# TaoMiner/joint-kg-recommender

Hardware: NVIDIA H100
Metric: scored (h,r,t) triples/s, TransE d=100 forward + margin loss + backward (higher is better)
Workload: dtype f32

## Files before the change

### joint-kg-recommender_b200/csrc/common.cuh

```cuda
#pragma once
#include <cuda_runtime.h>
#include <stdint.h>
#include "../../include/kgrec_b200.h"

namespace kgrec {

constexpr unsigned FULL = 0xffffffffu;
constexpr int kWarpsPerCta = 8;
constexpr int kThreads = kWarpsPerCta * 32;
constexpr int kMaxPref = 128;

void set_error(const char* fmt, ...);
#define KGREC_CUDA_OK(expr)                                                        \
  do {                                                                             \
    cudaError_t e__ = (expr);                                                      \
    if (e__ != cudaSuccess) {                                                      \
      kgrec::set_error("%s failed: %s (%s:%d)", #expr, cudaGetErrorString(e__),    \
                       __FILE__, __LINE__);                                        \
      return KGREC_ERR_CUDA;                                                       \
    }                                                                              \
  } while (0)
int sm_count();
float l2_keep_fraction(double table_bytes);

__device__ __forceinline__ float warp_sum(float v) {
#pragma unroll
  for (int o = 16; o > 0; o >>= 1) v += __shfl_xor_sync(FULL, v, o);
  return v;
}
__device__ __forceinline__ void warp_sum2(float& a, float& b) {
#pragma unroll
  for (int o = 16; o > 0; o >>= 1) {
    a += __shfl_xor_sync(FULL, a, o);
    b += __shfl_xor_sync(FULL, b, o);
  }
}
__device__ __forceinline__ float warp_max(float v) {
#pragma unroll
  for (int o = 16; o > 0; o >>= 1) v = fmaxf(v, __shfl_xor_sync(FULL, v, o));
  return v;
}

__device__ __forceinline__ float warp_reduce_scatter8(float (&v)[8], int lane) {
#pragma unroll
  for (int o = 16, n = 4; n > 0; o >>= 1, n >>= 1) {
    const bool up = (lane & o) != 0;
#pragma unroll
    for (int j = 0; j < 4; ++j) {
      if (j < n) {
        const float send = up ? v[j] : v[j + n];
        const float keep = up ? v[j + n] : v[j];
        v[j] = keep + __shfl_xor_sync(FULL, send, o);
      }
    }
  }
  float r = v[0];
  r += __shfl_xor_sync(FULL, r, 2);
  r += __shfl_xor_sync(FULL, r, 1);
  return r;
}

__device__ __forceinline__ int64_t load_idx(const void* p, int64_t i, int is64) {
  return is64 ? __ldg(reinterpret_cast<const long long*>(p) + i)
              : static_cast<int64_t>(__ldg(reinterpret_cast<const int*>(p) + i));
}
__device__ __forceinline__ int64_t checked(int64_t row, int64_t rows, int32_t* status) {
  if (static_cast<uint64_t>(row) >= static_cast<uint64_t>(rows)) {
    if (status) *status = 1;
    return 0;
  }
  return row;
}

__device__ __forceinline__ float4 ldg_f4(const float4* p) {
  float4 r;
  asm volatile("ld.global.nc.L1::no_allocate.v4.f32 {%0,%1,%2,%3}, [%4];"
               : "=f"(r.x), "=f"(r.y), "=f"(r.z), "=f"(r.w) : "l"(p));
  return r;
}
__device__ __forceinline__ void red_add_f4(float* p, float a, float b, float c, float d) {
  asm volatile("red.global.add.v4.f32 [%0], {%1,%2,%3,%4};" ::"l"(p), "f"(a), "f"(b), "f"(c), "f"(d)
               : "memory");
}

__device__ __forceinline__ void prefetch_l1(const void* p) { asm volatile("prefetch.global.L1 [%0];" ::"l"(p)); }

__device__ __forceinline__ uint32_t smem_u32(const void* p) { return static_cast<uint32_t>(__cvta_generic_to_shared(p)); }
__device__ __forceinline__ void mbar_init(uint64_t* bar, uint32_t count) {
  asm volatile("mbarrier.init.shared::cta.b64 [%0], %1;" ::"r"(smem_u32(bar)), "r"(count));
}
__device__ __forceinline__ void mbar_fence_init() { asm volatile("fence.mbarrier_init.release.cluster;" ::: "memory"); }
__device__ __forceinline__ void mbar_arrive(uint64_t* bar) {
  asm volatile("mbarrier.arrive.shared::cta.b64 _, [%0];" ::"r"(smem_u32(bar)) : "memory");
}
__device__ __forceinline__ void mbar_arrive_expect_tx(uint64_t* bar, uint32_t bytes) {
  asm volatile("mbarrier.arrive.expect_tx.shared::cta.b64 _, [%0], %1;" ::"r"(smem_u32(bar)), "r"(bytes) : "memory");
}
__device__ __forceinline__ bool mbar_try_wait(uint64_t* bar, uint32_t parity, uint32_t suspend_ns) {
  uint32_t ok;
  asm volatile(
      "{\n\t.reg .pred p;\n\t"
      "mbarrier.try_wait.parity.shared::cta.b64 p, [%1], %2, %3;\n\t"
      "selp.u32 %0, 1, 0, p;\n\t}"
      : "=r"(ok) : "r"(smem_u32(bar)), "r"(parity), "r"(suspend_ns) : "memory");
  return ok != 0;
}
__device__ __forceinline__ void mbar_wait(uint64_t* bar, uint32_t parity) {
  while (!mbar_try_wait(bar, parity, 20000u)) {}
}
__device__ __forceinline__ void bulk_g2s(void* dst, const void* src, uint32_t bytes, uint64_t* bar) {
  asm volatile("cp.async.bulk.shared::cluster.global.mbarrier::complete_tx::bytes [%0], [%1], %2, [%3];" ::"r"(
                   smem_u32(dst)),
               "l"(src), "r"(bytes), "r"(smem_u32(bar))
               : "memory");
}

__device__ __forceinline__ void fence_proxy_async_smem() { asm volatile("fence.proxy.async.shared::cta;" ::: "memory"); }
__device__ __forceinline__ float4 lds_f4(uint32_t addr) {
  float4 r;
  asm volatile("ld.shared.v4.f32 {%0,%1,%2,%3}, [%4];" : "=f"(r.x), "=f"(r.y), "=f"(r.z), "=f"(r.w) : "r"(addr));
  return r;
}

__device__ __forceinline__ uint64_t policy_evict_last(float fraction) {
  uint64_t p;
  asm volatile("createpolicy.fractional.L2::evict_last.L2::evict_unchanged.b64 %0, %1;" : "=l"(p) : "f"(fraction));
  return p;
}
__device__ __forceinline__ uint64_t policy_evict_first() {
  uint64_t p;
  asm volatile("createpolicy.fractional.L2::evict_first.b64 %0, 1.0;" : "=l"(p));
  return p;
}
__device__ __forceinline__ float4 ldg_f4_hint(const float4* p, uint64_t pol) {
  float4 r;
  asm volatile("ld.global.nc.L1::no_allocate.L2::cache_hint.v4.f32 {%0,%1,%2,%3}, [%4], %5;"
               : "=f"(r.x), "=f"(r.y), "=f"(r.z), "=f"(r.w) : "l"(p), "l"(pol));
  return r;
}
__device__ __forceinline__ void stg_f4_hint(float4* p, float a, float b, float c, float d, uint64_t pol) {
  asm volatile("st.global.L2::cache_hint.v4.f32 [%0], {%1,%2,%3,%4}, %5;" ::"l"(p), "f"(a), "f"(b), "f"(c), "f"(d), "l"(pol)
               : "memory");
}

template <int NCH, bool VEC>
struct Row {
  static constexpr int NE = NCH * 4;
  __device__ __forceinline__ static int elem(int lane, int e) {
    return VEC ? ((lane + 32 * (e >> 2)) * 4 + (e & 3)) : (lane + 32 * e);
  }
  __device__ __forceinline__ static void load(float (&v)[NE], const float* __restrict__ row, int d, int lane) {
    if (VEC) {
#pragma unroll
      for (int i = 0; i < NCH; ++i) {
        const int c = lane + 32 * i;
        float4 t = make_float4(0.f, 0.f, 0.f, 0.f);
        if (c * 4 < d) t = ldg_f4(reinterpret_cast<const float4*>(row) + c);
        v[4 * i] = t.x; v[4 * i + 1] = t.y; v[4 * i + 2] = t.z; v[4 * i + 3] = t.w;
      }
    } else {
#pragma unroll
      for (int e = 0; e < NE; ++e) {
        const int j = lane + 32 * e;
        v[e] = (j < d) ? __ldg(row + j) : 0.f;
      }
    }
  }
  __device__ __forceinline__ static void load_hint(float (&v)[NE], const float* __restrict__ row, int d, int lane, uint64_t pol) {
    static_assert(VEC, "cache-hinted loads are built for the 128-bit path");
#pragma unroll
    for (int i = 0; i < NCH; ++i) {
      const int c = lane + 32 * i;
      float4 t = make_float4(0.f, 0.f, 0.f, 0.f);
      if (c * 4 < d) t = ldg_f4_hint(reinterpret_cast<const float4*>(row) + c, pol);
      v[4 * i] = t.x; v[4 * i + 1] = t.y; v[4 * i + 2] = t.z; v[4 * i + 3] = t.w;
    }
  }
  __device__ __forceinline__ static void store_hint(float* __restrict__ row, const float (&v)[NE], int d, int lane, uint64_t pol) {
    static_assert(VEC, "cache-hinted stores are built for the 128-bit path");
#pragma unroll
    for (int i = 0; i < NCH; ++i) {
      const int c = lane + 32 * i;
      if (c * 4 < d) stg_f4_hint(reinterpret_cast<float4*>(row) + c, v[4 * i], v[4 * i + 1], v[4 * i + 2], v[4 * i + 3], pol);
    }
  }
  __device__ __forceinline__ static void load_s(float (&v)[NE], const float* row, int d, int lane) {
    if (VEC) {
#pragma unroll
      for (int i = 0; i < NCH; ++i) {
        const int c = lane + 32 * i;
        float4 t = make_float4(0.f, 0.f, 0.f, 0.f);
        if (c * 4 < d) t = reinterpret_cast<const float4*>(row)[c];
        v[4 * i] = t.x; v[4 * i + 1] = t.y; v[4 * i + 2] = t.z; v[4 * i + 3] = t.w;
      }
    } else {
#pragma unroll
      for (int e = 0; e < NE; ++e) {
        const int j = lane + 32 * e;
// ... 115 lines not shown
```

### joint-kg-recommender_b200/csrc/train_group.cu

```cuda
#include <cstdlib>
#include "train_dev.cuh"

namespace kgrec {

struct GroupArgs {
  kgrec_tables T;
  const void *ph, *pt, *pr;
  int is64;
  const int32_t* corrupt;
  LossCfg L;
  float keep;
};

__device__ __forceinline__ const float* row_ptr(const float* base, uint32_t row, uint32_t ld) {
  return base + static_cast<uint64_t>(row) * ld;
}

template <int FAM, int NCH>
struct GroupPos {
  using R = Row<NCH, true>;
  static constexpr int NE = R::NE;
  float h[NE], t[NE], w[NE];
  float base_h[NE];
  float base_t[NE];
// ... 466 lines not shown
        cpos += tt > 0.f ? 1.f : 0.f;
      } else {
        const float xx = prm * (sp - sn);
        lsum += fmaxf(-xx, 0.f) + log1pf(expf(-fabsf(xx)));
        const float dp = -prm / (1.f + expf(xx));
        cpos += dp;
        coef = dp * up;
      }
      if (FWD) return;
      const bool regx = REG && nx2 > 1.f;
      if (coef != 0.f || regx) {
        float4 gc = z4;
        if (coef != 0.f) {
          if (L1) {
            gc = make_float4(coef * ddist_term(e.x, 1), coef * ddist_term(e.y, 1), coef * ddist_term(e.z, 1), coef * ddist_term(e.w, 1));
          } else {
            const float c2 = 2.f * coef;
            gc = make_float4(c2 * e.x, c2 * e.y, c2 * e.z, c2 * e.w);
          }
          if (head) { accH.x -= gc.x; accH.y -= gc.y; accH.z -= gc.z; accH.w -= gc.w; }
          else { accT.x -= gc.x; accT.y -= gc.y; accT.z -= gc.z; accT.w -= gc.w; }
        }
        if (regx) { gc.x = fmaf(r2, x.x, gc.x); gc.y = fmaf(r2, x.y, gc.y); gc.z = fmaf(r2, x.z, gc.z); gc.w = fmaf(r2, x.w, gc.w); }
        if (act) {
          if (DENSE) red_add_f4(reinterpret_cast<float*>(gent_b + static_cast<uint64_t>(id) * d4), gc.x, gc.y, gc.z, gc.w);
          else stg_f4_hint(reinterpret_cast<float4*>(gent_b + goff), gc.x, gc.y, gc.z, gc.w, pol_stream);
        }
      } else if (!DENSE) {
        if (act) stg_f4_hint(reinterpret_cast<float4*>(gent_b + goff), 0.f, 0.f, 0.f, 0.f, pol_stream);
      }
      goff += d4;
    };

    for (int k = 0; k < K; k += 2) {
      if (k + 1 < K) {
        idb = ent_id(__shfl_sync(FULL, cv, k + 1), headb);
        if (act) xb = ldg_f4_hint(row(ent_b, idb), pol_keep);
      }
      negative(xa, heada, ida, k);
      if (k + 1 < K) {
        if (k + 2 < K) {
          ida = ent_id(__shfl_sync(FULL, cv, k + 2), heada);
          if (act) xa = ldg_f4_hint(row(ent_b, ida), pol_keep);
        }
        negative(xb, headb, idb, k + 1);
      }
    }
    const float cp = cpos * up;
    const float4 eps = make_float4(cp * ddist_term(ep.x, L1), cp * ddist_term(ep.y, L1), cp * ddist_term(ep.z, L1), cp * ddist_term(ep.w, L1));
    float4 gh = make_float4(accT.x + eps.x, accT.y + eps.y, accT.z + eps.z, accT.w + eps.w);
    float4 gt = make_float4(accH.x - eps.x, accH.y - eps.y, accH.z - eps.z, accH.w - eps.w);
    float4 gr = make_float4(accT.x - accH.x + eps.x, accT.y - accH.y + eps.y, accT.z - accH.z + eps.z, accT.w - accH.w + eps.w);
    if (REG) {
      const float mh = 1.f + n_tail, mt = 1.f + (static_cast<float>(K) - n_tail), mr = 1.f + static_cast<float>(K);
      lreg += mh * fmaxf(nh2 - 1.f, 0.f) + mt * fmaxf(nt2 - 1.f, 0.f) + mr * fmaxf(nr2 - 1.f, 0.f);
      const float ch = nh2 > 1.f ? mh * r2 : 0.f, ct = nt2 > 1.f ? mt * r2 : 0.f, cr = nr2 > 1.f ? mr * r2 : 0.f;
      gh.x = fmaf(ch, h.x, gh.x); gh.y = fmaf(ch, h.y, gh.y); gh.z = fmaf(ch, h.z, gh.z); gh.w = fmaf(ch, h.w, gh.w);
      gt.x = fmaf(ct, t.x, gt.x); gt.y = fmaf(ct, t.y, gt.y); gt.z = fmaf(ct, t.z, gt.z); gt.w = fmaf(ct, t.w, gt.w);
      gr.x = fmaf(cr, r.x, gr.x); gr.y = fmaf(cr, r.y, gr.y); gr.z = fmaf(cr, r.z, gr.z); gr.w = fmaf(cr, r.w, gr.w);
    }
    if (!BWD) {
      if (lane == 0) {
        pos_scores[j] = sp;
        group_loss[j] = lsum + (REG ? lreg : 0.f);
      }
      if (lane < K) neg_scores[static_cast<uint32_t>(j) * K + lane] = mys;
    }
    if (!FWD && act) {
      if (DENSE) {
        red_add_f4(reinterpret_cast<float*>(gent_b + static_cast<uint64_t>(ih0) * d4), gh.x, gh.y, gh.z, gh.w);
        red_add_f4(reinterpret_cast<float*>(gent_b + static_cast<uint64_t>(it0) * d4), gt.x, gt.y, gt.z, gt.w);
        red_add_f4(reinterpret_cast<float*>(grel_b + static_cast<uint64_t>(ir0) * d4), gr.x, gr.y, gr.z, gr.w);
      } else {
        const uint32_t g0 = static_cast<uint32_t>(j) * (2 + K) * d4;
        stg_f4_hint(reinterpret_cast<float4*>(gent_b + g0), gh.x, gh.y, gh.z, gh.w, pol_stream);
        stg_f4_hint(reinterpret_cast<float4*>(gent_b + g0 + d4), gt.x, gt.y, gt.z, gt.w, pol_stream);
        stg_f4_hint(reinterpret_cast<float4*>(grel_b + static_cast<uint32_t>(j) * d4), gr.x, gr.y, gr.z, gr.w, pol_stream);
      }
    }
  }
  if (bad && status) *status = 1;
}

template <bool L1, bool DENSE, bool MARGIN, int W>
__global__ void __launch_bounds__(W * 32, 1)
k_group_step_e_tma(const GroupArgs G, const float up0, float* __restrict__ pos_scores, float* __restrict__ neg_scores,
                   float* __restrict__ group_loss, const kgrec_grads Gr, int64_t* __restrict__ slot_ent,
                   int64_t* __restrict__ slot_rel, int32_t* status, const int S) {
  extern __shared__ __align__(128) unsigned char smem_raw[];
  const kgrec_tables& T = G.T;
  const LossCfg& L = G.L;
  const int lane = threadIdx.x & 31, wid = threadIdx.x >> 5;
  const int K = L.n_neg, n_rows = 3 + K;
  const int n_pos = static_cast<int>(L.n_pos);
  const uint32_t n_ent = static_cast<uint32_t>(T.n_ent);
  const uint32_t ld4 = static_cast<uint32_t>(T.ld) * 4u, d4 = static_cast<uint32_t>(T.dim) * 4u;
  const int bp = static_cast<int>(L.batch_pos < 0x7fffffff ? L.batch_pos : 0x7fffffff);
  const uint64_t pol_stream = policy_evict_first();
  const bool act = lane * 4 < T.dim;
  uint64_t* bars = reinterpret_cast<uint64_t*>(smem_raw) + wid * S;
  int32_t* ids_ring = reinterpret_cast<int32_t*>(smem_raw + static_cast<size_t>(W) * S * 8) + wid * S * 32;
  const uint32_t stage_bytes = static_cast<uint32_t>(n_rows) * d4;
  unsigned char* rows_base = smem_raw + ((static_cast<size_t>(W) * S * (8 + 128) + 127) & ~static_cast<size_t>(127)) +
                             static_cast<size_t>(wid) * S * stage_bytes;
  if (lane == 0)
    for (int s = 0; s < S; ++s) mbar_init(bars + s, 1);
  mbar_fence_init();
  __syncwarp();
  char* gent_b = reinterpret_cast<char*>(Gr.ent) + lane * 16;
  char* grel_b = reinterpret_cast<char*>(Gr.rel) + lane * 16;
  const float prm = L.param;
  const int stride = gridDim.x * W;
  const float4 z4 = make_float4(0.f, 0.f, 0.f, 0.f);
  bool bad = false;
  const void* pcol = lane == 0 ? G.ph : (lane == 1 ? G.pt : G.pr);

  auto issue = [&](int jj, int s) {
    int32_t v = 0;
    if (lane < 3) {
      const int64_t pv = load_idx(pcol, jj, G.is64);
      const int64_t lim = lane == 2 ? T.n_rel : T.n_ent;
      if (static_cast<uint64_t>(pv) >= static_cast<uint64_t>(lim)) bad = true; else v = static_cast<int32_t>(pv);
    } else if (lane < n_rows) {
      v = __ldg(G.corrupt + static_cast<uint32_t>(jj) * K + (lane - 3));
      const uint32_t id = static_cast<uint32_t>(v < 0 ? ~v : v);
      if (id >= n_ent) { bad = true; v = 0; }
    }
    ids_ring[s * 32 + lane] = v;
    if (lane == 0) mbar_arrive_expect_tx(bars + s, stage_bytes);
    __syncwarp();
    if (lane < n_rows) {
      const uint32_t id = lane < 3 ? static_cast<uint32_t>(v) : static_cast<uint32_t>(v < 0 ? ~v : v);
      const char* src = reinterpret_cast<const char*>(lane == 2 ? T.rel : T.ent) + static_cast<uint64_t>(id) * ld4;
      bulk_g2s(rows_base + static_cast<size_t>(s) * stage_bytes + static_cast<size_t>(lane) * d4, src, d4, bars + s);
    }
  };

  int j = blockIdx.x * W + wid;
  for (int s = 0, jj = j; s < S - 1 && jj < n_pos; ++s, jj += stride) issue(jj, s);
  for (int it = 0; j < n_pos; j += stride, ++it) {
    const int s = it % S;
    {
      const int jn = j + (S - 1) * stride;
      if (jn < n_pos) {
        fence_proxy_async_smem();
        __syncwarp();
        issue(jn, (it + S - 1) % S);
      }
    }
    mbar_wait(bars + s, static_cast<uint32_t>(it / S) & 1u);
    const int32_t myid = ids_ring[s * 32 + lane];
    const uint32_t st_addr = smem_u32(rows_base + static_cast<size_t>(s) * stage_bytes) + lane * 16;
    const uint32_t ih0 = static_cast<uint32_t>(__shfl_sync(FULL, myid, 0)), it0 = static_cast<uint32_t>(__shfl_sync(FULL, myid, 1)),
                   ir0 = static_cast<uint32_t>(__shfl_sync(FULL, myid, 2));
    if (slot_ent) {
      const uint32_t s0 = static_cast<uint32_t>(j) * (2 + K);
      if (lane < 2) slot_ent[s0 + lane] = myid;
      if (lane == 2) slot_rel[j] = myid;
      if (lane >= 3 && lane < n_rows) slot_ent[s0 + lane - 1] = myid < 0 ? ~myid : myid;
    }
    float4 h = z4, t = z4, r = z4;
    if (act) { h = lds_f4(st_addr); t = lds_f4(st_addr + d4); r = lds_f4(st_addr + 2 * d4); }
    float up = up0;
    if (!MARGIN) {
      const int b = j / bp;
      up /= static_cast<float>(min(bp, n_pos - b * bp)) * static_cast<float>(K);
    }
    const float4 bh = make_float4(h.x + r.x, h.y + r.y, h.z + r.z, h.w + r.w);
    const float4 bt = make_float4(t.x - r.x, t.y - r.y, t.z - r.z, t.w - r.w);
    const float4 ep = make_float4(bh.x - t.x, bh.y - t.y, bh.z - t.z, bh.w - t.w);
    const float sp = warp_sum(dist_term(ep.x, L1) + dist_term(ep.y, L1) + dist_term(ep.z, L1) + dist_term(ep.w, L1));
    float lsum = 0.f, cpos = 0.f, mys = 0.f;
    float4 accT = z4, accH = z4;
    uint32_t goff = (static_cast<uint32_t>(j) * (2 + K) + 2) * d4;
#pragma unroll 2
    for (int k = 0; k < K; ++k) {
      const int32_t c = __shfl_sync(FULL, myid, 3 + k);
      const bool head = c < 0;
      const uint32_t id = static_cast<uint32_t>(head ? ~c : c);
      float4 x = z4;
      if (act) x = lds_f4(st_addr + (3 + k) * d4);
      const float4 B = head ? bt : bh;
      const float4 e = make_float4(B.x - x.x, B.y - x.y, B.z - x.z, B.w - x.w);
      const float sn = warp_sum(L1 ? fabsf(e.x) + fabsf(e.y) + fabsf(e.z) + fabsf(e.w)
                                   : __fmaf_rn(e.w, e.w, __fmaf_rn(e.z, e.z, __fmaf_rn(e.x, e.x, __fmul_rn(e.y, e.y)))));
      if (lane == k) mys = sn;
      float coef;
      if (MARGIN) {
        const float tt = sp - sn + prm;
        lsum += fmaxf(tt, 0.f);
        coef = tt > 0.f ? up : 0.f;
        cpos += tt > 0.f ? 1.f : 0.f;
      } else {
        const float xx = prm * (sp - sn);
        lsum += fmaxf(-xx, 0.f) + log1pf(expf(-fabsf(xx)));
        const float dp = -prm / (1.f + expf(xx));
        cpos += dp;
        coef = dp * up;
      }
      if (coef != 0.f) {
        float4 gc;
        if (L1) {
          gc = make_float4(coef * ddist_term(e.x, 1), coef * ddist_term(e.y, 1), coef * ddist_term(e.z, 1), coef * ddist_term(e.w, 1));
        } else {
          const float c2 = 2.f * coef;
          gc = make_float4(c2 * e.x, c2 * e.y, c2 * e.z, c2 * e.w);
        }
        if (head) { accH.x -= gc.x; accH.y -= gc.y; accH.z -= gc.z; accH.w -= gc.w; }
        else { accT.x -= gc.x; accT.y -= gc.y; accT.z -= gc.z; accT.w -= gc.w; }
        if (act) {
          if (DENSE) red_add_f4(reinterpret_cast<float*>(gent_b + static_cast<uint64_t>(id) * d4), gc.x, gc.y, gc.z, gc.w);
          else stg_f4_hint(reinterpret_cast<float4*>(gent_b + goff), gc.x, gc.y, gc.z, gc.w, pol_stream);
        }
      } else if (!DENSE) {
        if (act) stg_f4_hint(reinterpret_cast<float4*>(gent_b + goff), 0.f, 0.f, 0.f, 0.f, pol_stream);
      }
      goff += d4;
    }
    const float cp = cpos * up;
    const float4 eps = make_float4(cp * ddist_term(ep.x, L1), cp * ddist_term(ep.y, L1), cp * ddist_term(ep.z, L1), cp * ddist_term(ep.w, L1));
    const float4 gh = make_float4(accT.x + eps.x, accT.y + eps.y, accT.z + eps.z, accT.w + eps.w);
    const float4 gt = make_float4(accH.x - eps.x, accH.y - eps.y, accH.z - eps.z, accH.w - eps.w);
    const float4 gr = make_float4(accT.x - accH.x + eps.x, accT.y - accH.y + eps.y, accT.z - accH.z + eps.z, accT.w - accH.w + eps.w);
    if (lane == 0) {
      pos_scores[j] = sp;
      group_loss[j] = lsum;
    }
    if (lane < K) neg_scores[static_cast<uint32_t>(j) * K + lane] = mys;
    if (act) {
      if (DENSE) {
        red_add_f4(reinterpret_cast<float*>(gent_b + static_cast<uint64_t>(ih0) * d4), gh.x, gh.y, gh.z, gh.w);
        red_add_f4(reinterpret_cast<float*>(gent_b + static_cast<uint64_t>(it0) * d4), gt.x, gt.y, gt.z, gt.w);
        red_add_f4(reinterpret_cast<float*>(grel_b + static_cast<uint64_t>(ir0) * d4), gr.x, gr.y, gr.z, gr.w);
      } else {
        const uint32_t g0 = static_cast<uint32_t>(j) * (2 + K) * d4;
        stg_f4_hint(reinterpret_cast<float4*>(gent_b + g0), gh.x, gh.y, gh.z, gh.w, pol_stream);
        stg_f4_hint(reinterpret_cast<float4*>(gent_b + g0 + d4), gt.x, gt.y, gt.z, gt.w, pol_stream);
        stg_f4_hint(reinterpret_cast<float4*>(grel_b + static_cast<uint32_t>(j) * d4), gr.x, gr.y, gr.z, gr.w, pol_stream);
      }
    }
  }
  if (bad && status) *status = 1;
}

template <bool L1, bool DENSE, bool MARGIN, int MINB, bool PF, bool REG, bool BWD, bool FWD = false>
__global__ void __launch_bounds__(kThreads, MINB)
k_group_step_h(const GroupArgs G, const float up0, const float* __restrict__ up_dev, float* __restrict__ pos_scores,
               float* __restrict__ neg_scores, float* __restrict__ group_loss, const kgrec_grads Gr,
               int64_t* __restrict__ slot_ent, int64_t* __restrict__ slot_rel, int32_t* status) {
  const kgrec_tables& T = G.T;
  const LossCfg& L = G.L;
  const int lane = threadIdx.x & 31, wid = threadIdx.x >> 5;
  const int K = L.n_neg;
  const int n_pos = static_cast<int>(L.n_pos);
  const uint32_t n_ent = static_cast<uint32_t>(T.n_ent);
  const uint32_t ld4 = static_cast<uint32_t>(T.ld) * 4u, d4 = static_cast<uint32_t>(T.dim) * 4u;
  const int bp = static_cast<int>(L.batch_pos < 0x7fffffff ? L.batch_pos : 0x7fffffff);
  const uint64_t pol_keep = policy_evict_last(G.keep), pol_stream = policy_evict_first();
  const bool act = lane * 4 < T.dim;
  const char* ent_b = reinterpret_cast<const char*>(T.ent) + lane * 16;
  const char* rel_b = reinterpret_cast<const char*>(T.rel) + lane * 16;
  const char* nrm_b = reinterpret_cast<const char*>(T.norm) + lane * 16;
  char* gent_b = reinterpret_cast<char*>(Gr.ent) + lane * 16;
  char* grel_b = reinterpret_cast<char*>(Gr.rel) + lane * 16;
  char* gnrm_b = reinterpret_cast<char*>(Gr.norm) + lane * 16;
  const float prm = L.param;
  const int stride = gridDim.x * kWarpsPerCta;
  const float4 z4 = make_float4(0.f, 0.f, 0.f, 0.f);
  auto row = [&](const char* base, uint32_t id) { return reinterpret_cast<const float4*>(base + static_cast<uint64_t>(id) * ld4); };
  auto dot4 = [](const float4& a, const float4& b) { return fmaf(a.x, b.x, fmaf(a.y, b.y, fmaf(a.z, b.z, a.w * b.w))); };
  bool bad = false;
  auto ent_id = [&](int32_t c, bool& head) {
    head = c < 0;
    uint32_t id = static_cast<uint32_t>(head ? ~c : c);
    if (id >= n_ent) { bad = true; id = 0; }
    return id;
  };
  int j = blockIdx.x * kWarpsPerCta + wid;
  const void* pcol = lane == 0 ? G.ph : (lane == 1 ? G.pt : G.pr);
  auto fetch_ids = [&](int jj, int32_t& cv, int64_t& pv) {
    cv = lane < K ? __ldg(G.corrupt + static_cast<uint32_t>(jj) * K + lane) : 0;
    pv = lane < 3 ? load_idx(pcol, jj, G.is64) : 0;
  };
  int32_t cv = 0, cvn = 0;
  int64_t pv = 0, pvn = 0;
  if (j < n_pos) fetch_ids(j, cvn, pvn);
  for (; j < n_pos; j += stride) {
    cv = cvn;
    pv = pvn;
    const int jn = j + stride;
    if (jn < n_pos) fetch_ids(jn, cvn, pvn);
    const int64_t vh = __shfl_sync(FULL, pv, 0), vt = __shfl_sync(FULL, pv, 1), vr = __shfl_sync(FULL, pv, 2);
    uint32_t ih = static_cast<uint32_t>(vh), it = static_cast<uint32_t>(vt), ir = static_cast<uint32_t>(vr);
    if (static_cast<uint64_t>(vh) >= static_cast<uint64_t>(T.n_ent)) { bad = true; ih = 0; }
    if (static_cast<uint64_t>(vt) >= static_cast<uint64_t>(T.n_ent)) { bad = true; it = 0; }
    if (static_cast<uint64_t>(vr) >= static_cast<uint64_t>(T.n_rel)) { bad = true; ir = 0; }
    if (slot_ent) {
      const uint32_t s0 = static_cast<uint32_t>(j) * (2 + K);
      if (lane < 2) slot_ent[s0 + lane] = pv;
      if (lane == 2) slot_rel[j] = pv;
      if (lane < K) slot_ent[s0 + 2 + lane] = cv < 0 ? ~cv : cv;
    }
    float4 h = z4, t = z4, r = z4, w = z4, xa = z4, xb = z4;
    bool heada, headb = false;
    uint32_t ida = ent_id(__shfl_sync(FULL, cv, 0), heada), idb = 0;
    if (act) {
      h = ldg_f4_hint(row(ent_b, ih), pol_keep);
      t = ldg_f4_hint(row(ent_b, it), pol_keep);
      r = ldg_f4_hint(row(rel_b, ir), pol_keep);
      w = ldg_f4_hint(row(nrm_b, ir), pol_keep);
      xa = ldg_f4_hint(row(ent_b, ida), pol_keep);
    }
    if (PF && lane >= 2 && lane < K) {
      const uint32_t pid = static_cast<uint32_t>(cv < 0 ? ~cv : cv);
      if (pid < n_ent) {
        const char* pr = reinterpret_cast<const char*>(T.ent) + static_cast<uint64_t>(pid) * ld4;
        for (uint32_t o = 0; o < d4; o += 128) prefetch_l1(pr + o);
      }
    }
    float up = up0;
    if (BWD && up_dev) up *= __ldg(up_dev + j / bp);
    if (!MARGIN) {
// ... 901 lines not shown
    return KGREC_ERR_INVALID;
  }
  if ((slot_ent_ids == nullptr) != (slot_rel_ids == nullptr)) { set_error("slot_ent_ids and slot_rel_ids go together"); return KGREC_ERR_INVALID; }
  if (pl.fam == FAM_R) {
    if (reg_flags) { set_error("fused regularisers are built for TransE / TransH"); return KGREC_ERR_UNSUPPORTED; }
    if (pl.nch != 1 || n_neg > 14) { set_error("TransR step kernel: embedding_size <= 128 and at most 14 negatives per positive"); return KGREC_ERR_UNSUPPORTED; }
    if (n_pos == 0) return KGREC_OK;
    const GroupArgs GA{*tables, ph, pt, pr, idx_bytes == 8, corrupt, LossCfg{loss_kind, margin_or_target, n_neg, n_pos, batch_pos}, 1.f};
    float* gl = static_cast<float*>(workspace);
    cudaStream_t s2 = static_cast<cudaStream_t>(stream);
    int32_t* order = reinterpret_cast<int32_t*>(gl + n_pos);
    int32_t* cursor = order + n_pos;
    {
      const char* env = group_step_env();
      if (env && env[0] == 'u') order = nullptr;
    }
    if (order) {
      KGREC_CUDA_OK(cudaMemsetAsync(cursor, 0, sizeof(int32_t) * tables->n_rel, s2));
      const int gs = static_cast<int>((n_pos + 255) / 256 < sm_count() * 4 ? (n_pos + 255) / 256 : sm_count() * 4);
      k_rel_hist<<<gs, 256, 0, s2>>>(pr, idx_bytes == 8, static_cast<int>(n_pos), tables->n_rel, cursor);
      k_rel_scan<<<1, 1024, 0, s2>>>(cursor, tables->n_rel);
      k_rel_scatter<<<gs, 256, 0, s2>>>(pr, idx_bytes == 8, static_cast<int>(n_pos), tables->n_rel, cursor, order);
    }
    const bool mg = loss_kind == KGREC_LOSS_MARGIN;
    const char* env_r = group_step_env();
    const bool long_runs = n_pos >= 4 * tables->n_rel || (env_r && env_r[0] == 'r');
    if (tables->dim >= 32 && long_runs && !(env_r && (env_r[0] == 'w' || env_r[0] == 'u'))) {
      const int d = tables->dim, NC = d / 4, pitch = run_pitch(d), qf = d / 32;
      auto smem_for = [&](int rb) { return (2 * static_cast<size_t>(d) + 2 * 64 * rb) * pitch * 4 + 3 * 64 * rb * 8 + 72 * 4; };
      const int rb = (NC <= 27 && smem_for(2) <= 220 * 1024) ? 2 : 1;
      const size_t smem = smem_for(rb);
      const int64_t want = (n_pos + 3) / 4;
      const int grid = static_cast<int>(want < sm_count() ? want : sm_count());
#define CALL_RUN(QAV, QBV, QFV, RBV)                                                                                     \
  {                                                                                                                      \
    auto kern = mg ? k_run_step_r<QAV, QBV, QFV, RBV, true> : k_run_step_r<QAV, QBV, QFV, RBV, false>;                   \
    KGREC_CUDA_OK(cudaFuncSetAttribute(kern, cudaFuncAttributeMaxDynamicSharedMemorySize, static_cast<int>(smem)));       \
    kern<<<grid, kThreads, smem, s2>>>(GA, grad_loss, pos_scores, neg_scores, gl, *grads, slot_ent_ids, slot_rel_ids, status, order); \
  }
      if (NC <= 16) { if (qf <= 1) CALL_RUN(1, 1, 1, 2) else CALL_RUN(1, 1, 2, 2) }
      else if (NC <= 27) { if (qf <= 2) CALL_RUN(1, 3, 2, 2) else CALL_RUN(1, 3, 3, 2) }
      else { if (qf <= 3) CALL_RUN(2, 2, 3, 1) else CALL_RUN(2, 2, 4, 1) }
#undef CALL_RUN
    } else {
    const int64_t want = (n_pos + kWarpsPerCta - 1) / kWarpsPerCta;
    const int grid_r = static_cast<int>(want < sm_count() ? want : sm_count());
    const int nvt = n_neg <= 2 ? 4 : (n_neg <= 10 ? 12 : 16);
    const size_t smem = static_cast<size_t>(kWarpsPerCta) * (static_cast<size_t>(nvt) * (tables->dim / 4) + static_cast<size_t>(tables->dim) * (nvt / 4)) * 16;
#define CALL_R(NVTV, MV)                                                                                             \
  {                                                                                                                  \
    auto kern = k_group_step_r<NVTV, MV>;                                                                            \
    KGREC_CUDA_OK(cudaFuncSetAttribute(kern, cudaFuncAttributeMaxDynamicSharedMemorySize, static_cast<int>(smem)));   \
    kern<<<grid_r, kThreads, smem, s2>>>(GA, grad_loss, pos_scores, neg_scores, gl, *grads, slot_ent_ids, slot_rel_ids, status, order); \
  }
    if (nvt == 4) { if (mg) CALL_R(4, true) else CALL_R(4, false) }
    else if (nvt == 12) { if (mg) CALL_R(12, true) else CALL_R(12, false) }
    else { if (mg) CALL_R(16, true) else CALL_R(16, false) }
#undef CALL_R
    }
    KGREC_CUDA_OK(cudaGetLastError());
    const int64_t nbt = (n_pos + batch_pos - 1) / batch_pos;
    k_batch_loss<<<static_cast<unsigned>(nbt), 256, 0, s2>>>(gl, GA.L, loss);
    KGREC_CUDA_OK(cudaGetLastError());
    return KGREC_OK;
  }
  if (n_pos == 0) return KGREC_OK;
  const GroupArgs G{*tables, ph, pt, pr, idx_bytes == 8, corrupt, LossCfg{loss_kind, margin_or_target, n_neg, n_pos, batch_pos},
                    l2_keep_fraction(static_cast<double>(tables->n_ent) * tables->ld * sizeof(float))};
  float* group_loss = static_cast<float*>(workspace);
  cudaStream_t st = static_cast<cudaStream_t>(stream);
  if (reg_flags != 0 && reg_flags != 1) { set_error("reg_flags must be 0 or 1"); return KGREC_ERR_INVALID; }
  if (reg_flags && loss_kind != KGREC_LOSS_MARGIN) { set_error("fused regularisers go with the margin loss (the KG drivers' loss)"); return KGREC_ERR_UNSUPPORTED; }
  const char* env = group_step_env();
  const bool small32 = n_neg <= 32 && static_cast<double>(n_pos) * (2 + n_neg) * tables->dim * 4 < 4.0e9 &&
                       static_cast<double>(n_pos) * n_neg < 2.0e9;
  const bool tma = pl.fam == FAM_E && pl.nch == 1 && small32 && grads->mode == 0 && !reg_flags && n_neg <= 29 &&
                   tables->ld == tables->dim && !(env && (env[0] == '0' || env[0] == 'n' || env[0] == '3')) &&
                   group_step_tma_smem(tables->dim, n_neg) <= 225 * 1024 &&
                   n_pos >= static_cast<int64_t>(kTmaStages) * kTmaWarps * sm_count();
  if (tma) {
    const size_t smem = group_step_tma_smem(tables->dim, n_neg);
    int64_t ctas = (n_pos + kTmaWarps - 1) / kTmaWarps;
    if (ctas > sm_count()) ctas = sm_count();
#define CALL_T(L1V, MV)                                                                                                 \
  {                                                                                                                     \
    auto kern = k_group_step_e_tma<L1V, false, MV, kTmaWarps>;                                                          \
    KGREC_CUDA_OK(cudaFuncSetAttribute(kern, cudaFuncAttributeMaxDynamicSharedMemorySize, static_cast<int>(smem)));      \
    kern<<<static_cast<int>(ctas), kTmaWarps * 32, smem, st>>>(G, grad_loss, pos_scores, neg_scores, group_loss, *grads, slot_ent_ids, slot_rel_ids, status, kTmaStages); \
  }
    const bool mg = loss_kind == KGREC_LOSS_MARGIN;
    if (tables->l1) { if (mg) CALL_T(true, true) else CALL_T(true, false) }
    else { if (mg) CALL_T(false, true) else CALL_T(false, false) }
#undef CALL_T
  } else if (pl.fam == FAM_E && pl.nch == 1 && small32 && !(env && env[0] == '0')) {
#define CALL_E(L1V, DV, MV)                                                                                      \
  {                                                                                                              \
    if (env && env[0] == 'n')                                                                                    \
      k_group_step_e<L1V, DV, MV, 4, false, false, false><<<grid_for(n_pos), kThreads, 0, st>>>(G, grad_loss, nullptr, pos_scores, neg_scores, group_loss, *grads, slot_ent_ids, slot_rel_ids, status); \
    else if (env && env[0] == '3')                                                                               \
      k_group_step_e<L1V, DV, MV, 3, false, false, false><<<grid_for(n_pos), kThreads, 0, st>>>(G, grad_loss, nullptr, pos_scores, neg_scores, group_loss, *grads, slot_ent_ids, slot_rel_ids, status); \
    else if (MV && reg_flags)                                                                                    \
      k_group_step_e<L1V, DV, true, 4, true, true, false><<<grid_for(n_pos), kThreads, 0, st>>>(G, grad_loss, nullptr, pos_scores, neg_scores, group_loss, *grads, slot_ent_ids, slot_rel_ids, status); \
    else                                                                                                         \
      k_group_step_e<L1V, DV, MV, 4, true, false, false><<<grid_for(n_pos), kThreads, 0, st>>>(G, grad_loss, nullptr, pos_scores, neg_scores, group_loss, *grads, slot_ent_ids, slot_rel_ids, status); \
  }
    const bool dn = grads->mode == 1, mg = loss_kind == KGREC_LOSS_MARGIN;
    if (tables->l1) { if (dn) { if (mg) CALL_E(true, true, true) else CALL_E(true, true, false) } else { if (mg) CALL_E(true, false, true) else CALL_E(true, false, false) } }
    else { if (dn) { if (mg) CALL_E(false, true, true) else CALL_E(false, true, false) } else { if (mg) CALL_E(false, false, true) else CALL_E(false, false, false) } }
#undef CALL_E
  } else if (pl.fam == FAM_H && pl.nch == 1 && small32 && !(env && env[0] == '0')) {
#define CALL_H(L1V, DV, MV)                                                                                      \
  {                                                                                                              \
    if (env && env[0] == 'n')                                                                                    \
      k_group_step_h<L1V, DV, MV, 3, false, false, false><<<grid_for(n_pos), kThreads, 0, st>>>(G, grad_loss, nullptr, pos_scores, neg_scores, group_loss, *grads, slot_ent_ids, slot_rel_ids, status); \
    else if (env && env[0] == '2')                                                                               \
      k_group_step_h<L1V, DV, MV, 2, false, false, false><<<grid_for(n_pos), kThreads, 0, st>>>(G, grad_loss, nullptr, pos_scores, neg_scores, group_loss, *grads, slot_ent_ids, slot_rel_ids, status); \
    else if (MV && reg_flags)                                                                                    \
      k_group_step_h<L1V, DV, true, 3, true, true, false><<<grid_for(n_pos), kThreads, 0, st>>>(G, grad_loss, nullptr, pos_scores, neg_scores, group_loss, *grads, slot_ent_ids, slot_rel_ids, status); \
    else                                                                                                         \
      k_group_step_h<L1V, DV, MV, 3, true, false, false><<<grid_for(n_pos), kThreads, 0, st>>>(G, grad_loss, nullptr, pos_scores, neg_scores, group_loss, *grads, slot_ent_ids, slot_rel_ids, status); \
  }
    const bool dn = grads->mode == 1, mg = loss_kind == KGREC_LOSS_MARGIN;
    if (tables->l1) { if (dn) { if (mg) CALL_H(true, true, true) else CALL_H(true, true, false) } else { if (mg) CALL_H(true, false, true) else CALL_H(true, false, false) } }
    else { if (dn) { if (mg) CALL_H(false, true, true) else CALL_H(false, true, false) } else { if (mg) CALL_H(false, false, true) else CALL_H(false, false, false) } }
#undef CALL_H
  } else {
    if (reg_flags) { set_error("fused regularisers are built for the d <= 128 margin-loss step kernels only"); return KGREC_ERR_UNSUPPORTED; }
#define CALL(FAMV, NCHV)                                                                                        \
  if (tables->l1) k_group_step<FAMV, NCHV, true><<<grid_for(n_pos), kThreads, 0, st>>>(G, grad_loss, pos_scores, neg_scores, group_loss, *grads, status); \
  else k_group_step<FAMV, NCHV, false><<<grid_for(n_pos), kThreads, 0, st>>>(G, grad_loss, pos_scores, neg_scores, group_loss, *grads, status);
  KGREC_GROUP_DISPATCH(CALL)
#undef CALL
    if (slot_ent_ids) {
      const int64_t total = n_pos * (2 + static_cast<int64_t>(n_neg));
      const int64_t ctas = (total + 255) / 256, cap = static_cast<int64_t>(sm_count()) * 16;
      k_group_slot_ids<<<static_cast<unsigned>(ctas < cap ? ctas : cap), 256, 0, st>>>(ph, pt, pr, idx_bytes == 8, corrupt, n_pos, n_neg,
                                                                                         slot_ent_ids, slot_rel_ids);
    }
  }
  KGREC_CUDA_OK(cudaGetLastError());
  const int64_t n_batches = (n_pos + batch_pos - 1) / batch_pos;
  k_batch_loss<<<static_cast<unsigned>(n_batches), 256, 0, st>>>(group_loss, G.L, loss);
  KGREC_CUDA_OK(cudaGetLastError());
  return KGREC_OK;
}
```

Measured before the change: 2.888 billion.

## Batch negative-score reductions with warp reduce-scatter and deepen TMA prefetch pipeline

Measured after the change: 2.978 billion, median of 6. 3.1% higher.

```diff
diff --git a/joint-kg-recommender_b200/csrc/common.cuh b/joint-kg-recommender_b200/csrc/common.cuh
--- a/joint-kg-recommender_b200/csrc/common.cuh
+++ b/joint-kg-recommender_b200/csrc/common.cuh
@@ -60,6 +60,27 @@
   return r;
 }
 
+template <int N>
+__device__ __forceinline__ float warp_reduce_scatter(float (&v)[N], int lane) {
+  static_assert(N == 16 || N == 32, "16 or 32 partials");
+#pragma unroll
+  for (int l = 0; l < (N == 32 ? 5 : 4); ++l) {
+    const int o = 16 >> l, n = N >> (l + 1);
+    const bool up = (lane & o) != 0;
+#pragma unroll
+    for (int i = 0; i < N / 2; ++i) {
+      if (i < n) {
+        const float send = up ? v[i] : v[i + n];
+        const float keep = up ? v[i + n] : v[i];
+        v[i] = keep + __shfl_xor_sync(FULL, send, o);
+      }
+    }
+  }
+  float r = v[0];
+  if (N == 16) r += __shfl_xor_sync(FULL, r, 1);
+  return r;
+}
+
 __device__ __forceinline__ int64_t load_idx(const void* p, int64_t i, int is64) {
   return is64 ? __ldg(reinterpret_cast<const long long*>(p) + i)
               : static_cast<int64_t>(__ldg(reinterpret_cast<const int*>(p) + i));
@@ -114,6 +135,12 @@
                "l"(src), "r"(bytes), "r"(smem_u32(bar))
                : "memory");
 }
+__device__ __forceinline__ void bulk_g2s_hint(void* dst, const void* src, uint32_t bytes, uint64_t* bar, uint64_t pol) {
+  asm volatile("cp.async.bulk.shared::cluster.global.mbarrier::complete_tx::bytes.L2::cache_hint [%0], [%1], %2, [%3], %4;" ::"r"(
+                   smem_u32(dst)),
+               "l"(src), "r"(bytes), "r"(smem_u32(bar)), "l"(pol)
+               : "memory");
+}
 
 __device__ __forceinline__ void fence_proxy_async_smem() { asm volatile("fence.proxy.async.shared::cta;" ::: "memory"); }
 __device__ __forceinline__ float4 lds_f4(uint32_t addr) {
diff --git a/joint-kg-recommender_b200/csrc/train_group.cu b/joint-kg-recommender_b200/csrc/train_group.cu
--- a/joint-kg-recommender_b200/csrc/train_group.cu
+++ b/joint-kg-recommender_b200/csrc/train_group.cu
@@ -572,11 +572,14 @@
   if (bad && status) *status = 1;
 }
 
-template <bool L1, bool DENSE, bool MARGIN, int W>
+template <bool L1, bool MARGIN, int W, int NS>
 __global__ void __launch_bounds__(W * 32, 1)
 k_group_step_e_tma(const GroupArgs G, const float up0, float* __restrict__ pos_scores, float* __restrict__ neg_scores,
                    float* __restrict__ group_loss, const kgrec_grads Gr, int64_t* __restrict__ slot_ent,
                    int64_t* __restrict__ slot_rel, int32_t* status, const int S) {
+  static_assert(NS == 16 || NS == 32, "a group's scores are reduced over 16 or 32 slots");
+  constexpr int NK = NS - 1;
+  constexpr bool KEEP = NS == 16;
   extern __shared__ __align__(128) unsigned char smem_raw[];
   const kgrec_tables& T = G.T;
   const LossCfg& L = G.L;
@@ -586,7 +589,7 @@
   const uint32_t n_ent = static_cast<uint32_t>(T.n_ent);
   const uint32_t ld4 = static_cast<uint32_t>(T.ld) * 4u, d4 = static_cast<uint32_t>(T.dim) * 4u;
   const int bp = static_cast<int>(L.batch_pos < 0x7fffffff ? L.batch_pos : 0x7fffffff);
-  const uint64_t pol_stream = policy_evict_first();
+  const uint64_t pol_keep = policy_evict_last(G.keep), pol_stream = policy_evict_first();
   const bool act = lane * 4 < T.dim;
   uint64_t* bars = reinterpret_cast<uint64_t*>(smem_raw) + wid * S;
   int32_t* ids_ring = reinterpret_cast<int32_t*>(smem_raw + static_cast<size_t>(W) * S * 8) + wid * S * 32;
@@ -605,14 +608,17 @@
   bool bad = false;
   const void* pcol = lane == 0 ? G.ph : (lane == 1 ? G.pt : G.pr);
 
-  auto issue = [&](int jj, int s) {
+  auto fetch = [&](int jj) -> int64_t {
+    if (lane < 3) return load_idx(pcol, jj, G.is64);
+    return lane < n_rows ? static_cast<int64_t>(__ldg(G.corrupt + static_cast<uint32_t>(jj) * K + (lane - 3))) : 0;
+  };
+  auto issue = [&](int64_t pv, int s) {
     int32_t v = 0;
     if (lane < 3) {
-      const int64_t pv = load_idx(pcol, jj, G.is64);
       const int64_t lim = lane == 2 ? T.n_rel : T.n_ent;
       if (static_cast<uint64_t>(pv) >= static_cast<uint64_t>(lim)) bad = true; else v = static_cast<int32_t>(pv);
     } else if (lane < n_rows) {
-      v = __ldg(G.corrupt + static_cast<uint32_t>(jj) * K + (lane - 3));
+      v = static_cast<int32_t>(pv);
       const uint32_t id = static_cast<uint32_t>(v < 0 ? ~v : v);
       if (id >= n_ent) { bad = true; v = 0; }
     }
@@ -622,91 +628,128 @@
     if (lane < n_rows) {
       const uint32_t id = lane < 3 ? static_cast<uint32_t>(v) : static_cast<uint32_t>(v < 0 ? ~v : v);
       const char* src = reinterpret_cast<const char*>(lane == 2 ? T.rel : T.ent) + static_cast<uint64_t>(id) * ld4;
-      bulk_g2s(rows_base + static_cast<size_t>(s) * stage_bytes + static_cast<size_t>(lane) * d4, src, d4, bars + s);
+      bulk_g2s_hint(rows_base + static_cast<size_t>(s) * stage_bytes + static_cast<size_t>(lane) * d4, src, d4, bars + s,
+                    pol_keep);
     }
   };
+  auto sub4 = [](const float4& a, const float4& b) { return make_float4(a.x - b.x, a.y - b.y, a.z - b.z, a.w - b.w); };
+  auto dist4 = [](const float4& e) {
+    return L1 ? fabsf(e.x) + fabsf(e.y) + fabsf(e.z) + fabsf(e.w)
+              : __fmaf_rn(e.w, e.w, __fmaf_rn(e.z, e.z, __fmaf_rn(e.x, e.x, __fmul_rn(e.y, e.y))));
+  };
 
   int j = blockIdx.x * W + wid;
-  for (int s = 0, jj = j; s < S - 1 && jj < n_pos; ++s, jj += stride) issue(jj, s);
+  for (int s = 0, jj = j; s < S && jj < n_pos; ++s, jj += stride) issue(fetch(jj), s);
+  int64_t nv = j + S * stride < n_pos ? fetch(j + S * stride) : 0;
   for (int it = 0; j < n_pos; j += stride, ++it) {
     const int s = it % S;
-    {
-      const int jn = j + (S - 1) * stride;
-      if (jn < n_pos) {
-        fence_proxy_async_smem();
-        __syncwarp();
-        issue(jn, (it + S - 1) % S);
-      }
-    }
     mbar_wait(bars + s, static_cast<uint32_t>(it / S) & 1u);
     const int32_t myid = ids_ring[s * 32 + lane];
     const uint32_t st_addr = smem_u32(rows_base + static_cast<size_t>(s) * stage_bytes) + lane * 16;
-    const uint32_t ih0 = static_cast<uint32_t>(__shfl_sync(FULL, myid, 0)), it0 = static_cast<uint32_t>(__shfl_sync(FULL, myid, 1)),
-                   ir0 = static_cast<uint32_t>(__shfl_sync(FULL, myid, 2));
+    auto release = [&]() {
+      const int jr = j + S * stride;
+      if (jr < n_pos) {
+        fence_proxy_async_smem();
+        __syncwarp();
+        issue(nv, s);
+        if (jr + stride < n_pos) nv = fetch(jr + stride);
+      }
+    };
+    float4 h = z4, t = z4, r = z4;
+    float4 x[KEEP ? NK : 1];
+    if (act) { h = lds_f4(st_addr); t = lds_f4(st_addr + d4); r = lds_f4(st_addr + 2 * d4); }
+    if (KEEP) {
+#pragma unroll
+      for (int k = 0; k < NK; ++k) {
+        x[k] = z4;
+        if (k < K && act) x[k] = lds_f4(st_addr + (3 + k) * d4);
+      }
+      release();
+    }
+    const uint32_t hm = __ballot_sync(FULL, myid < 0) >> 3;
     if (slot_ent) {
       const uint32_t s0 = static_cast<uint32_t>(j) * (2 + K);
       if (lane < 2) slot_ent[s0 + lane] = myid;
       if (lane == 2) slot_rel[j] = myid;
       if (lane >= 3 && lane < n_rows) slot_ent[s0 + lane - 1] = myid < 0 ? ~myid : myid;
     }
-    float4 h = z4, t = z4, r = z4;
-    if (act) { h = lds_f4(st_addr); t = lds_f4(st_addr + d4); r = lds_f4(st_addr + 2 * d4); }
+    const float4 bh = make_float4(h.x + r.x, h.y + r.y, h.z + r.z, h.w + r.w);
+    const float4 bt = make_float4(t.x - r.x, t.y - r.y, t.z - r.z, t.w - r.w);
+    const float4 ep = sub4(bh, t);
+    auto residual = [&](int k) {
+      float4 xk = z4;
+      if (KEEP) xk = x[k];
+      else if (act) xk = lds_f4(st_addr + (3 + k) * d4);
+      return sub4((hm >> k) & 1u ? bt : bh, xk);
+    };
+    float p[NS];
+#pragma unroll
+    for (int k = 0; k < NS; ++k) p[k] = 0.f;
+    p[NS - 1] = dist4(ep);
+#pragma unroll
+    for (int k = 0; k < NK; ++k) {
+      if (k < K) {
+        const float4 e = residual(k);
+        if (KEEP) x[k] = e;
+        p[k] = dist4(e);
+      }
+    }
+    const float sv = warp_reduce_scatter<NS>(p, lane);
+    const float sp = __shfl_sync(FULL, sv, 31);
+    const int kl = NS == 32 ? lane : lane >> 1;
+    const bool mine = kl < K && (NS == 32 || (lane & 1) == 0);
+    if (mine) neg_scores[static_cast<uint32_t>(j) * K + kl] = sv;
     float up = up0;
     if (!MARGIN) {
       const int b = j / bp;
       up /= static_cast<float>(min(bp, n_pos - b * bp)) * static_cast<float>(K);
     }
-    const float4 bh = make_float4(h.x + r.x, h.y + r.y, h.z + r.z, h.w + r.w);
-    const float4 bt = make_float4(t.x - r.x, t.y - r.y, t.z - r.z, t.w - r.w);
-    const float4 ep = make_float4(bh.x - t.x, bh.y - t.y, bh.z - t.z, bh.w - t.w);
-    const float sp = warp_sum(dist_term(ep.x, L1) + dist_term(ep.y, L1) + dist_term(ep.z, L1) + dist_term(ep.w, L1));
-    float lsum = 0.f, cpos = 0.f, mys = 0.f;
+    float lt, dq = 0.f;
+    uint32_t am = 0;
+    if (MARGIN) {
+      const float tt = sp - sv + prm;
+      lt = fmaxf(tt, 0.f);
+      am = __ballot_sync(FULL, mine && tt > 0.f);
+    } else {
+      const float xx = prm * (sp - sv);
+      lt = fmaxf(-xx, 0.f) + log1pf(expf(-fabsf(xx)));
+      dq = -prm / (1.f + expf(xx));
+    }
+    float lsum = 0.f, cpos = MARGIN ? static_cast<float>(__popc(am)) : 0.f;
     float4 accT = z4, accH = z4;
     uint32_t goff = (static_cast<uint32_t>(j) * (2 + K) + 2) * d4;
-#pragma unroll 2
-    for (int k = 0; k < K; ++k) {
-      const int32_t c = __shfl_sync(FULL, myid, 3 + k);
-      const bool head = c < 0;
-      const uint32_t id = static_cast<uint32_t>(head ? ~c : c);
-      float4 x = z4;
-      if (act) x = lds_f4(st_addr + (3 + k) * d4);
-      const float4 B = head ? bt : bh;
-      const float4 e = make_float4(B.x - x.x, B.y - x.y, B.z - x.z, B.w - x.w);
-      const float sn = warp_sum(L1 ? fabsf(e.x) + fabsf(e.y) + fabsf(e.z) + fabsf(e.w)
-                                   : __fmaf_rn(e.w, e.w, __fmaf_rn(e.z, e.z, __fmaf_rn(e.x, e.x, __fmul_rn(e.y, e.y)))));
-      if (lane == k) mys = sn;
-      float coef;
-      if (MARGIN) {
-        const float tt = sp - sn + prm;
-        lsum += fmaxf(tt, 0.f);
-        coef = tt > 0.f ? up : 0.f;
-        cpos += tt > 0.f ? 1.f : 0.f;
-      } else {
-        const float xx = prm * (sp - sn);
-        lsum += fmaxf(-xx, 0.f) + log1pf(expf(-fabsf(xx)));
-        const float dp = -prm / (1.f + expf(xx));
-        cpos += dp;
-        coef = dp * up;
-      }
-      if (coef != 0.f) {
-        float4 gc;
-        if (L1) {
-          gc = make_float4(coef * ddist_term(e.x, 1), coef * ddist_term(e.y, 1), coef * ddist_term(e.z, 1), coef * ddist_term(e.w, 1));
+#pragma unroll
+    for (int k = 0; k < NK; ++k) {
+      if (k < K) {
+        constexpr int kw = NS == 32 ? 1 : 2;
+        lsum += __shfl_sync(FULL, lt, kw * k);
+        float coef;
+        if (MARGIN) {
+          coef = (am >> (kw * k)) & 1u ? up : 0.f;
         } else {
-          const float c2 = 2.f * coef;
-          gc = make_float4(c2 * e.x, c2 * e.y, c2 * e.z, c2 * e.w);
-        }
-        if (head) { accH.x -= gc.x; accH.y -= gc.y; accH.z -= gc.z; accH.w -= gc.w; }
-        else { accT.x -= gc.x; accT.y -= gc.y; accT.z -= gc.z; accT.w -= gc.w; }
-        if (act) {
-          if (DENSE) red_add_f4(reinterpret_cast<float*>(gent_b + static_cast<uint64_t>(id) * d4), gc.x, gc.y, gc.z, gc.w);
-          else stg_f4_hint(reinterpret_cast<float4*>(gent_b + goff), gc.x, gc.y, gc.z, gc.w, pol_stream);
-        }
-      } else if (!DENSE) {
-        if (act) stg_f4_hint(reinterpret_cast<float4*>(gent_b + goff), 0.f, 0.f, 0.f, 0.f, pol_stream);
-      }
-      goff += d4;
-    }
+          const float dp = __shfl_sync(FULL, dq, kw * k);
+          cpos += dp;
+          coef = dp * up;
+        }
+        if (coef != 0.f) {
+          const float4 e = KEEP ? x[k] : residual(k);
+          float4 gc;
+          if (L1) {
+            gc = make_float4(coef * ddist_term(e.x, 1), coef * ddist_term(e.y, 1), coef * ddist_term(e.z, 1), coef * ddist_term(e.w, 1));
+          } else {
+            const float c2 = 2.f * coef;
+            gc = make_float4(c2 * e.x, c2 * e.y, c2 * e.z, c2 * e.w);
+          }
+          if ((hm >> k) & 1u) { accH.x -= gc.x; accH.y -= gc.y; accH.z -= gc.z; accH.w -= gc.w; }
+          else { accT.x -= gc.x; accT.y -= gc.y; accT.z -= gc.z; accT.w -= gc.w; }
+          if (act) stg_f4_hint(reinterpret_cast<float4*>(gent_b + goff), gc.x, gc.y, gc.z, gc.w, pol_stream);
+        } else if (act) {
+          stg_f4_hint(reinterpret_cast<float4*>(gent_b + goff), 0.f, 0.f, 0.f, 0.f, pol_stream);
+        }
+        goff += d4;
+      }
+    }
+    if (!KEEP) release();
     const float cp = cpos * up;
     const float4 eps = make_float4(cp * ddist_term(ep.x, L1), cp * ddist_term(ep.y, L1), cp * ddist_term(ep.z, L1), cp * ddist_term(ep.w, L1));
     const float4 gh = make_float4(accT.x + eps.x, accT.y + eps.y, accT.z + eps.z, accT.w + eps.w);
@@ -716,18 +759,11 @@
       pos_scores[j] = sp;
       group_loss[j] = lsum;
     }
-    if (lane < K) neg_scores[static_cast<uint32_t>(j) * K + lane] = mys;
     if (act) {
-      if (DENSE) {
-        red_add_f4(reinterpret_cast<float*>(gent_b + static_cast<uint64_t>(ih0) * d4), gh.x, gh.y, gh.z, gh.w);
-        red_add_f4(reinterpret_cast<float*>(gent_b + static_cast<uint64_t>(it0) * d4), gt.x, gt.y, gt.z, gt.w);
-        red_add_f4(reinterpret_cast<float*>(grel_b + static_cast<uint64_t>(ir0) * d4), gr.x, gr.y, gr.z, gr.w);
-      } else {
-        const uint32_t g0 = static_cast<uint32_t>(j) * (2 + K) * d4;
-        stg_f4_hint(reinterpret_cast<float4*>(gent_b + g0), gh.x, gh.y, gh.z, gh.w, pol_stream);
-        stg_f4_hint(reinterpret_cast<float4*>(gent_b + g0 + d4), gt.x, gt.y, gt.z, gt.w, pol_stream);
-        stg_f4_hint(reinterpret_cast<float4*>(grel_b + static_cast<uint32_t>(j) * d4), gr.x, gr.y, gr.z, gr.w, pol_stream);
-      }
+      const uint32_t g0 = static_cast<uint32_t>(j) * (2 + K) * d4;
+      stg_f4_hint(reinterpret_cast<float4*>(gent_b + g0), gh.x, gh.y, gh.z, gh.w, pol_stream);
+      stg_f4_hint(reinterpret_cast<float4*>(gent_b + g0 + d4), gt.x, gt.y, gt.z, gt.w, pol_stream);
+      stg_f4_hint(reinterpret_cast<float4*>(grel_b + static_cast<uint32_t>(j) * d4), gr.x, gr.y, gr.z, gr.w, pol_stream);
     }
   }
   if (bad && status) *status = 1;
@@ -1795,15 +1831,17 @@
     const size_t smem = group_step_tma_smem(tables->dim, n_neg);
     int64_t ctas = (n_pos + kTmaWarps - 1) / kTmaWarps;
     if (ctas > sm_count()) ctas = sm_count();
-#define CALL_T(L1V, MV)                                                                                                 \
+#define CALL_T(L1V, MV, NSV)                                                                                            \
   {                                                                                                                     \
-    auto kern = k_group_step_e_tma<L1V, false, MV, kTmaWarps>;                                                          \
+    auto kern = k_group_step_e_tma<L1V, MV, kTmaWarps, NSV>;                                                            \
     KGREC_CUDA_OK(cudaFuncSetAttribute(kern, cudaFuncAttributeMaxDynamicSharedMemorySize, static_cast<int>(smem)));      \
     kern<<<static_cast<int>(ctas), kTmaWarps * 32, smem, st>>>(G, grad_loss, pos_scores, neg_scores, group_loss, *grads, slot_ent_ids, slot_rel_ids, status, kTmaStages); \
   }
+#define CALL_TN(L1V, MV) { if (n_neg < 16) CALL_T(L1V, MV, 16) else CALL_T(L1V, MV, 32) }
     const bool mg = loss_kind == KGREC_LOSS_MARGIN;
-    if (tables->l1) { if (mg) CALL_T(true, true) else CALL_T(true, false) }
-    else { if (mg) CALL_T(false, true) else CALL_T(false, false) }
+    if (tables->l1) { if (mg) CALL_TN(true, true) else CALL_TN(true, false) }
+    else { if (mg) CALL_TN(false, true) else CALL_TN(false, false) }
+#undef CALL_TN
 #undef CALL_T
   } else if (pl.fam == FAM_E && pl.nch == 1 && small32 && !(env && env[0] == '0')) {
 #define CALL_E(L1V, DV, MV)                                                                                      \
```
